# gitvicky/CP-PRE

Hardware: AMD Instinct MI355X
Metric: residual-cells/s (PRE eval+calibrate) (higher is better)
Workload: dtype f32

## Files before the change

### cp_pre_amd/csrc/calib.hip

```cpp
#include "common.h"
#include "guarded_divide.h"

#pragma clang fp contract(off)

namespace {

__global__ void __launch_bounds__(256) absdiff_kernel(const float *__restrict__ a, const float *__restrict__ b,
                                                      float *__restrict__ out, long long n)
{
    const bool vec = !(((uintptr_t)a | (uintptr_t)out | (uintptr_t)(b ? b : a)) & 15);
    long long done = 0;
    if (vec) {
        const long long n4 = n / 4;
        const float4 *a4 = reinterpret_cast<const float4 *>(a);
        const float4 *b4 = reinterpret_cast<const float4 *>(b);
        float4 *o4 = reinterpret_cast<float4 *>(out);
        for (long long blk = blockIdx.x; blk * 1024 < n4; blk += gridDim.x) {
            const long long i = blk * 1024 + threadIdx.x;
            float4 v[4], w[4];
#pragma unroll
            for (int u = 0; u < 4; ++u)
                if (i + u * 256 < n4) v[u] = a4[i + u * 256];
            if (b) {
#pragma unroll
// ... 100 lines not shown
        constexpr int width = 64 * H / US;
#pragma unroll
        for (int k = 0; k < H; ++k) {
            if constexpr (width == 32) {
                const ms_u32x2 r = __builtin_amdgcn_permlane32_swap(m[k], m[H + k], false, false);
                m[k] = max(r.x, r.y);
            } else if constexpr (width == 16) {
                const ms_u32x2 r = __builtin_amdgcn_permlane16_swap(m[k], m[H + k], false, false);
                m[k] = max(r.x, r.y);
            } else {
                const bool up = lane & width;
                const unsigned int mine = up ? m[H + k] : m[k], send = up ? m[k] : m[H + k];
                m[k] = max(mine, dpp_xor<width>(send));
            }
        }
        ms_butterfly<US, H / 2>(m, lane);
    }
}

__device__ __forceinline__ float ms_cell(const float *p, unsigned int cb, unsigned int plane_bytes)
{
    const __amdgpu_buffer_rsrc_t r = __builtin_amdgcn_make_buffer_rsrc(const_cast<float *>(p), 0, plane_bytes, 0x00020000);
    return __uint_as_float(__builtin_amdgcn_raw_buffer_load_b32(r, (int)cb, 0, 0));
}

template <int TCH, int US, bool FULL>
__device__ __forceinline__ void ms_load(const float *__restrict__ au, unsigned int c, long long row_stride, long long plane, int i, int nt,
                                        float (&v)[US][TCH])
{
#pragma unroll
    for (int u = 0; u < US; ++u)
#pragma unroll
        for (int t = 0; t < TCH; ++t)
            v[u][t] = ms_cell(au + ((i + u) * row_stride + (FULL || TCH == 1 || t < nt ? t : nt - 1) * plane), c, (unsigned int)plane * 4u);
}

struct MsStage { unsigned int (*m)[17]; unsigned int *row0; long long nseg_left; };
template <int TCH, int US, bool FULL>
__device__ __forceinline__ void ms_use(const float (&v)[US][TCH], int i, int nt, bool scored, double (&s)[TCH], double (&q)[TCH],
                                       unsigned int *__restrict__ seg, long long seg_stride, const MsStage *stage = nullptr)
{
    unsigned int m[US];
#pragma unroll
    for (int u = 0; u < US; ++u) {
        int mp = 0;
        unsigned int mn = 0u;
#pragma unroll
        for (int t = 0; t < TCH; ++t) {
            const float x = (FULL || TCH == 1 || t < nt) ? v[u][t] : 0.f;
            const double d = (double)x;
            s[t] += d;
            q[t] = __builtin_fma(d, d, q[t]);
            mp = max(mp, (int)__float_as_uint(x));
            mn = max(mn, __float_as_uint(x));
        }
        m[u] = max((unsigned int)mp, mn & 0x7fffffffu);
        m[u] = scored ? m[u] : 0u;
    }
    const int lane = threadIdx.x & 63;
    if constexpr (US == 1) {
        m[0] = wave_max_u32_to_lane63(m[0]);
        if (lane == 63 && seg) seg[i * seg_stride] = m[0];
    } else {
        ms_butterfly<US, US / 2>(m, lane);
        if constexpr (64 / US > 8) m[0] = max(m[0], dpp_xor<8>(m[0]));
        if constexpr (64 / US > 4) m[0] = max(m[0], dpp_xor<4>(m[0]));
        m[0] = max(m[0], dpp_xor<2>(m[0]));
        m[0] = max(m[0], dpp_xor<1>(m[0]));
        if (US == 16 && stage) {
            if ((lane & 3) == 0) stage->m[threadIdx.x >> 6][lane >> 2] = m[0];
            __syncthreads();
            if (threadIdx.x < 256) {
                const int smp = (int)(threadIdx.x >> 4), sg = (int)(threadIdx.x & 15);
                if (sg < stage->nseg_left) stage->row0[(i + smp) * seg_stride + sg] = stage->m[sg][smp];
            }
            __syncthreads();
        } else if ((lane & (64 / US - 1)) == 0) seg[(i + lane / (64 / US)) * seg_stride] = m[0];
    }
}

template <int TCH, int US, bool FULL>
__device__ __forceinline__ void ms_samples(const float *__restrict__ au, unsigned int c, long long row_stride, long long plane, int i0, int i1,
                                           int nt, bool scored, double (&s)[TCH], double (&q)[TCH], unsigned int *__restrict__ seg,
                                           long long seg_stride, const MsStage *stage = nullptr)
{
    int i = i0;
    if constexpr (US == 1) {
        float va[1][TCH], vb[1][TCH];
        if (i < i1) ms_load<TCH, 1, FULL>(au, c, row_stride, plane, i, nt, va);
        for (; i < i1; i += 2) {
            ms_load<TCH, 1, FULL>(au, c, row_stride, plane, min(i + 1, i1 - 1), nt, vb);
            ms_use<TCH, 1, FULL>(va, i, nt, scored, s, q, seg, seg_stride);
            if (i + 1 >= i1) break;
            ms_load<TCH, 1, FULL>(au, c, row_stride, plane, min(i + 2, i1 - 1), nt, va);
            ms_use<TCH, 1, FULL>(vb, i + 1, nt, scored, s, q, seg, seg_stride);
        }
    } else {
        float v[US][TCH], w[US][TCH], v1[1][TCH];
        const int ilast = i0 + (i1 - i0) / US * US - US;
        if (i + US <= i1) ms_load<TCH, US, FULL>(au, c, row_stride, plane, i, nt, v);
        for (; i + US <= i1; i += 2 * US) {
            ms_load<TCH, US, FULL>(au, c, row_stride, plane, min(i + US, ilast), nt, w);
            ms_use<TCH, US, FULL>(v, i, nt, scored, s, q, seg, seg_stride, stage);
            if (i + 2 * US > i1) { i += US; break; }
            ms_load<TCH, US, FULL>(au, c, row_stride, plane, min(i + 2 * US, ilast), nt, v);
            ms_use<TCH, US, FULL>(w, i + US, nt, scored, s, q, seg, seg_stride, stage);
        }
        for (; i < i1; ++i) {
            ms_load<TCH, 1, FULL>(au, c, row_stride, plane, i, nt, v1);
            ms_use<TCH, 1, FULL>(v1, i, nt, scored, s, q, seg, seg_stride);
        }
    }
}

template <int TCH, int US>
__global__ void __launch_bounds__(US == 16 && MS_STAGE ? 1024 : 256)
moments_segmax_kernel(const float *__restrict__ a, long long row_stride, int n, int T, int X,
                                                             int Y, int cx, int cy, int rows_per_split, double *__restrict__ sum,
                                                             double *__restrict__ sumsq, unsigned int *__restrict__ segmax)
{
    const long long plane = (long long)X * Y, cl = (long long)blockIdx.x * blockDim.x + threadIdx.x;
    if (!(US == 16 && MS_STAGE) && (cl & ~63LL) >= plane) return;
    const bool live = cl < plane;
    const long long c = live ? cl : plane - 1;
    const int x = (int)(c / Y), y = (int)(c - (long long)x * Y);
    const long long nseg = (plane + 63) / 64;
    const bool scored = live && x >= cx && x < X - cx && y >= cy && y < Y - cy;
    const int i0 = blockIdx.y * rows_per_split, i1 = min(n, i0 + rows_per_split);
    const int tc = blockIdx.z, TC = gridDim.z, t0 = tc * MS_TMAX, nt = min(TCH, T - t0);
    const float *au = a + (long long)t0 * plane;
    const long long seg_stride = (long long)TC * nseg;
    unsigned int *seg = segmax + (long long)tc * nseg + (cl >> 6);
    double s[TCH], q[TCH];
#pragma unroll
    for (int t = 0; t < TCH; ++t) s[t] = q[t] = 0.0;
    const unsigned int cb = (unsigned int)c * 4u;
    __shared__ unsigned int stage_m[US == 16 ? 16 : 1][17];
    MsStage st{stage_m, segmax + (long long)tc * nseg + (long long)blockIdx.x * (blockDim.x >> 6),
               nseg - (long long)blockIdx.x * (blockDim.x >> 6)};
    const MsStage *stage = (US == 16 && MS_STAGE) ? &st : nullptr;
    if (US == 16 && MS_STAGE && (cl & ~63LL) >= plane) seg = nullptr;
    if (nt == TCH) ms_samples<TCH, US, true>(au, cb, row_stride, plane, i0, i1, nt, scored, s, q, seg, seg_stride, stage);
    else ms_samples<TCH, US, false>(au, cb, row_stride, plane, i0, i1, nt, scored, s, q, seg, seg_stride, stage);
    sum += (long long)t0 * plane + c;
    sumsq += (long long)t0 * plane + c;
#pragma unroll
    for (int t = 0; t < TCH; ++t)
        if (t < nt && live) {
            if (gridDim.y == 1) { sum[t * plane] += s[t]; sumsq[t * plane] += q[t]; }
            else { atomicAdd(&sum[t * plane], s[t]); atomicAdd(&sumsq[t * plane], q[t]); }
        }
}

constexpr int MS4_US = 8;
constexpr int MS4_CG = 4;
constexpr int MS4_NT = 256 * MS4_CG, MS4_NW = 4 * MS4_CG;
constexpr int MS4_WANT = 256;
constexpr int MS4_AUX = 2;
typedef unsigned int ms4_u32x4 __attribute__((ext_vector_type(4)));

__device__ __forceinline__ void ms4_barrier()
{
    __builtin_amdgcn_fence(__ATOMIC_RELEASE, "workgroup", "local");
    __builtin_amdgcn_s_barrier();
    __builtin_amdgcn_fence(__ATOMIC_ACQUIRE, "workgroup", "local");
}

__device__ __forceinline__ void ms4_load(const float *au, unsigned int cb, long long row_stride, long long plane, int i, int nt,
                                         ms4_u32x4 (&v)[4])
{
#pragma unroll
    for (int k = 0; k < 4; ++k) {
        const __amdgpu_buffer_rsrc_t r = __builtin_amdgcn_make_buffer_rsrc(
            const_cast<float *>(au + ((long long)i * row_stride + k * plane)), 0, k < nt ? (unsigned int)plane * 4u : 0u, 0x00020000);
        v[k] = __builtin_amdgcn_raw_buffer_load_b128(r, (int)cb, 0, MS4_AUX);
    }
}

__device__ __forceinline__ unsigned int ms4_use(const ms4_u32x4 (&v)[4], const bool (&scored)[4], double (&s)[4][4], double (&q)[4][4])
{
    unsigned int m = 0u;
#pragma unroll
    for (int j = 0; j < 4; ++j) {
        int mp = 0;
        unsigned int mn = 0u;
#pragma unroll
        for (int k = 0; k < 4; ++k) {
            const unsigned int b = v[k][j];
            const double d = (double)__uint_as_float(b);
            s[k][j] += d;
            q[k][j] = __builtin_fma(d, d, q[k][j]);
            mp = max(mp, (int)b);
            mn = max(mn, b);
        }
        const unsigned int mc = max((unsigned int)mp, mn & 0x7fffffffu);
        m = max(m, scored[j] ? mc : 0u);
    }
    return m;
}

__device__ __forceinline__ void ms4_sample(const ms4_u32x4 (&v)[4], const bool (&scored)[4], double (&s)[4][4], double (&q)[4][4],
                                           unsigned int (&slot)[MS4_NW][4], int w, int lane)
{
    unsigned int m = ms4_use(v, scored, s, q);
    m = max(m, (unsigned int)__builtin_amdgcn_update_dpp(0, (int)m, 0x111, 0xf, 0xf, true));
    m = max(m, (unsigned int)__builtin_amdgcn_update_dpp(0, (int)m, 0x112, 0xf, 0xf, true));
    m = max(m, (unsigned int)__builtin_amdgcn_update_dpp(0, (int)m, 0x114, 0xf, 0xf, true));
    m = max(m, (unsigned int)__builtin_amdgcn_update_dpp(0, (int)m, 0x118, 0xf, 0xf, true));
    if ((lane & 15) == 15) slot[w][lane >> 4] = m;
}

__device__ __forceinline__ void ms4_samples(const float *au, unsigned int cb, long long row_stride, long long plane, int i0, int i1,
                                            int nt, const bool (&scored)[4], double (&s)[4][4], double (&q)[4][4],
                                            unsigned int (*stage)[MS4_US][MS4_NW][4], unsigned int *row0, int nseg_left,
                                            long long seg_stride)
{
    const int w = __builtin_amdgcn_readfirstlane((int)(threadIdx.x >> 6)), lane = (int)(threadIdx.x & 63);
    ms4_u32x4 va[4], vb[4];
    ms4_load(au, cb, row_stride, plane, i0, nt, va);
    int b = 0;
    for (int ib = i0; ib < i1; ib += MS4_US, b ^= 1) {
        const int cnt = min(MS4_US, i1 - ib);
#pragma unroll
        for (int u = 0; u < MS4_US; u += 2) {
            ms4_load(au, cb, row_stride, plane, min(ib + u + 1, i1 - 1), nt, vb);
            if (u < cnt) ms4_sample(va, scored, s, q, stage[b][u], w, lane);
            ms4_load(au, cb, row_stride, plane, min(ib + u + 2, i1 - 1), nt, va);
            if (u + 1 < cnt) ms4_sample(vb, scored, s, q, stage[b][u + 1], w, lane);
        }
        ms4_barrier();
        if (threadIdx.x < MS4_US * MS4_NW) {
            const int smp = (int)(threadIdx.x / MS4_NW), sg = (int)(threadIdx.x % MS4_NW), cg = sg >> 2, r = sg & 3;
            const unsigned int m = max(max(stage[b][smp][4 * cg][r], stage[b][smp][4 * cg + 1][r]),
                                       max(stage[b][smp][4 * cg + 2][r], stage[b][smp][4 * cg + 3][r]));
            if (smp < cnt && sg < nseg_left) row0[(long long)(ib + smp) * seg_stride + sg] = m;
        }
    }
}

__global__ void __launch_bounds__(MS4_NT) moments_segmax4_kernel(const float *__restrict__ a, long long row_stride, int n, int T,
                                                               int X, int Y, int cx, int cy, int rows_per_split,
                                                               double *__restrict__ sum, double *__restrict__ sumsq,
                                                               unsigned int *__restrict__ segmax)
{
    const long long plane = (long long)X * Y;
    const int w = __builtin_amdgcn_readfirstlane((int)(threadIdx.x >> 6)), lane = (int)(threadIdx.x & 63);
    const long long cl = (long long)blockIdx.x * MS4_NT + (w >> 2) * 256 + lane * 4;
    const bool live = cl < plane;
    const long long c = live ? cl : plane - 4;
    bool scored[4];
#pragma unroll
    for (int j = 0; j < 4; ++j) {
        const int x = (int)((c + j) / Y), y = (int)(c + j - (long long)x * Y);
        scored[j] = live && x >= cx && x < X - cx && y >= cy && y < Y - cy;
    }
    const long long nseg = (plane + 63) / 64;
    const int i0 = blockIdx.y * rows_per_split, i1 = min(n, i0 + rows_per_split);
    const int tc = blockIdx.z, TC = gridDim.z, t0 = tc * MS_TMAX + 4 * (w & 3), nt = min(4, T - t0);
    const float *au = a + (long long)min(t0, T - 1) * plane;
    const long long seg_stride = (long long)TC * nseg;
    unsigned int *row0 = segmax + (long long)tc * nseg + (long long)blockIdx.x * MS4_NW;
    const int nseg_left = (int)min((long long)MS4_NW, nseg - (long long)blockIdx.x * MS4_NW);
    double s[4][4], q[4][4];
#pragma unroll
    for (int k = 0; k < 4; ++k)
#pragma unroll
        for (int j = 0; j < 4; ++j) s[k][j] = q[k][j] = 0.0;
    __shared__ unsigned int stage[2][MS4_US][MS4_NW][4];
    const unsigned int cb = (unsigned int)c * 4u;
    ms4_samples(au, cb, row_stride, plane, i0, i1, nt, scored, s, q, stage, row0, nseg_left, seg_stride);
    if (!live) return;
#pragma unroll
    for (int k = 0; k < 4; ++k)
        if (k < nt) {
            double *ps = sum + (long long)(t0 + k) * plane + c, *pq = sumsq + (long long)(t0 + k) * plane + c;
#pragma unroll
            for (int j = 0; j < 4; ++j) {
                if (gridDim.y == 1) { ps[j] += s[k][j]; pq[j] += q[k][j]; }
                else { atomicAdd(&ps[j], s[k][j]); atomicAdd(&pq[j], q[k][j]); }
            }
        }
}

__global__ void __launch_bounds__(256) std_from_moments_kernel(const double *__restrict__ sum, const double *__restrict__ sumsq,
                                                               double n_total, long long M, float eps, float *__restrict__ mod)
{
    const long long c = (long long)blockIdx.x * blockDim.x + threadIdx.x;
    if (c >= M) return;
    const double mean = sum[c] / n_total;
    double var = sumsq[c] / n_total - mean * mean;
    var = var < 0.0 ? 0.0 : var;
    mod[c] = (float)sqrt(var) + eps;
}

__device__ __forceinline__ float wave_max(float v)
{
#pragma unroll
    for (int o = 32; o > 0; o >>= 1) v = fmaxf(v, __shfl_xor(v, o));
    return v;
}

constexpr int JS_RB = 32;
#ifndef JS_TARGET_CELLS
#define JS_TARGET_CELLS 65536
#endif
__device__ __forceinline__ void js_update(float av, float sv, float &m, float &thr, bool &nan)
{
    guarded_max_update(av, sv, m, thr, nan);
}

__global__ void __launch_bounds__(256) joint_score_kernel(const float *__restrict__ a, const float *__restrict__ b,
                                                          const float *__restrict__ mod, int T, int X, int Y,
                                                          int ct, int cx, int cy, int groups, int smp_fastest,
                                                          const unsigned int *__restrict__ only, float *__restrict__ scores)
{
    const long long plane = (long long)X * Y, vol = plane * T;
    const int smp = smp_fastest ? blockIdx.x : blockIdx.y;
    const unsigned int cblk = smp_fastest ? blockIdx.y : blockIdx.x;
    if (only && !only[smp]) return;
    const float *pa = a + smp * vol, *pb = b ? b + smp * vol : nullptr;
    const long long nrows = (long long)T * X;
    const bool vec = (Y % 4 == 0) && !(((uintptr_t)a | (uintptr_t)mod | (uintptr_t)(b ? b : a)) & 15);
    __shared__ unsigned int rowmask;
    __shared__ float red[4];
    float m = 0.f, thr = 0.f;
    bool any = false, nan = false;
    for (int gi = 0; gi < groups; ++gi) {
    const long long r0 = ((long long)cblk * groups + gi) * JS_RB;
    if (r0 >= nrows) break;
    __syncthreads();
    if (threadIdx.x < 64) {
        const long long r = r0 + threadIdx.x;
        bool ok = threadIdx.x < JS_RB && r < nrows;
        if (ok) {
            const int t = (int)(r / X), x = (int)(r % X);
            ok = !(t < ct || t >= T - ct || x < cx || x >= X - cx);
        }
        const unsigned long long bm = __ballot(ok);
        if (threadIdx.x == 0) rowmask = (unsigned int)bm;
    }
    __syncthreads();
    const unsigned int rows = rowmask;
    any = any || rows != 0u;
    if (rows && vec) {
        const int Y4 = Y / 4, dr = 256 / Y4, dy = 256 % Y4;
        int row = threadIdx.x / Y4, y4 = threadIdx.x % Y4;
        while (row < JS_RB) {
            if ((rows >> row) & 1u) {
                const long long o = (r0 + row) * Y + 4 * y4;
                float4 v = *reinterpret_cast<const float4 *>(pa + o);
                if (pb) { const float4 w = *reinterpret_cast<const float4 *>(pb + o); v = make_float4(v.x - w.x, v.y - w.y, v.z - w.z, v.w - w.w); }
                const float4 sg = *reinterpret_cast<const float4 *>(mod + o);
                const float av[4] = {fabsf(v.x), fabsf(v.y), fabsf(v.z), fabsf(v.w)};
                const float sv[4] = {sg.x, sg.y, sg.z, sg.w};
                const int y = 4 * y4;
#pragma unroll
                for (int k = 0; k < 4; ++k)
                    if (y + k >= cy && y + k < Y - cy) js_update(av[k], sv[k], m, thr, nan);
            }
            y4 += dy;
            row += dr;
            if (y4 >= Y4) { y4 -= Y4; ++row; }
        }
    } else if (rows) {
        const int dr = 256 / Y, dy = 256 % Y;
        int row = threadIdx.x / Y, y = threadIdx.x % Y;
        while (row < JS_RB) {
            if (((rows >> row) & 1u) && y >= cy && y < Y - cy) {
                const long long o = (r0 + row) * Y + y;
                float v = pa[o];
                if (pb) v -= pb[o];
                js_update(fabsf(v), mod[o], m, thr, nan);
            }
            y += dy;
            row += dr;
            if (y >= Y) { y -= Y; ++row; }
        }
    }
    }
    m = wave_max(m);
    if (__ballot(nan)) m = __uint_as_float(0x7fc00000u);
    if ((threadIdx.x & 63) == 0) red[threadIdx.x >> 6] = m;
    __syncthreads();
    if (threadIdx.x == 0 && any) {
        const unsigned int u = max(max(__float_as_uint(red[0]), __float_as_uint(red[1])),
                                   max(__float_as_uint(red[2]), __float_as_uint(red[3])));
        atomicMax(reinterpret_cast<unsigned int *>(scores) + smp, u);
    }
}

constexpr int JSF_CELLS = 8192;
__global__ void __launch_bounds__(256) joint_score_flat_kernel(const float *__restrict__ a, const float *__restrict__ b,
                                                               const float *__restrict__ mod, int T, int X, int Y, int ct,
                                                               int cx, int cy, const unsigned int *__restrict__ only,
                                                               float *__restrict__ scores)
{
    const long long vol = (long long)T * X * Y;
    const int smp = blockIdx.x;
    if (only && !only[smp]) return;
    const float4 *pa = reinterpret_cast<const float4 *>(a + smp * vol);
    const float4 *pb = b ? reinterpret_cast<const float4 *>(b + smp * vol) : nullptr;
    const float4 *pm = reinterpret_cast<const float4 *>(mod);
    const unsigned int c0 = blockIdx.y * (unsigned)JSF_CELLS;
    __shared__ float red[4];
    float m = 0.f, thr = 0.f;
    bool nan = false;
    unsigned int f = c0 + 4u * threadIdx.x;
    const unsigned int row0 = f / (unsigned)Y;
    int y0 = (int)(f - row0 * (unsigned)Y), x0 = (int)(row0 % (unsigned)X), t0 = (int)(row0 / (unsigned)X);
    const int dy = 1024 % Y, drow = 1024 / Y, dx = drow % X, dt = drow / X;
    for (int k = 0; k < JSF_CELLS / 1024 && f < (unsigned)vol; ++k, f += 1024u) {
        float4 v = pa[f >> 2];
        if (pb) { const float4 w = pb[f >> 2]; v = make_float4(v.x - w.x, v.y - w.y, v.z - w.z, v.w - w.w); }
        const float4 sg = pm[f >> 2];
        const float av[4] = {fabsf(v.x), fabsf(v.y), fabsf(v.z), fabsf(v.w)};
        const float sv[4] = {sg.x, sg.y, sg.z, sg.w};
        int y = y0, x = x0, t = t0;
#pragma unroll
        for (int j = 0; j < 4; ++j) {
            const bool in = t >= ct && t < T - ct && x >= cx && x < X - cx && y >= cy && y < Y - cy;
            if (in) js_update(av[j], sv[j], m, thr, nan);
            if (++y == Y) { y = 0; if (++x == X) { x = 0; ++t; } }
        }
        y0 += dy;
        const int carry = y0 >= Y;
        y0 -= carry ? Y : 0;
        x0 += dx + carry;
        const int cx2 = x0 >= X;
        x0 -= cx2 ? X : 0;
        t0 += dt + cx2;
    }
    m = wave_max(m);
    if (__ballot(nan)) m = __uint_as_float(0x7fc00000u);
    if ((threadIdx.x & 63) == 0) red[threadIdx.x >> 6] = m;
// ... 198 lines not shown
                } else if (hit) {
                    atomicAdd(&hist[d], 1u);
                }
            }
        };
        const float4 *s4 = reinterpret_cast<const float4 *>(s);
        for (long long i = threadIdx.x; i < N8; i += blockDim.x) {
            const float4 a = s4[2 * i], b = s4[2 * i + 1];
            count(a.x); count(a.y); count(a.z); count(a.w);
            count(b.x); count(b.y); count(b.z); count(b.w);
        }
        for (long long i = 8 * N8 + threadIdx.x; i < N; i += blockDim.x) count(s[i]);
        __syncthreads();
        if (threadIdx.x < 64) {
            const unsigned int c0 = hist[4 * lane], c1 = hist[4 * lane + 1], c2 = hist[4 * lane + 2], c3 = hist[4 * lane + 3];
            long long incl = (long long)c0 + c1 + c2 + c3;
#pragma unroll
            for (int o = 1; o < 64; o <<= 1) {
                const long long up = __shfl_up(incl, o);
                if (lane >= o) incl += up;
            }
            long long excl = incl - ((long long)c0 + c1 + c2 + c3);
            const bool mine = (excl <= rank && rank < incl) || (lane == 63 && rank >= incl);
            if (mine) {
                unsigned int d = 4 * lane;
                if (rank >= excl + c0) { excl += c0; ++d; if (rank >= excl + c1) { excl += c1; ++d; if (rank >= excl + c2) { excl += c2; ++d; } } }
                sh_prefix = prefix | (d << shift);
                sh_rank = rank - excl;
            }
        }
        __syncthreads();
        prefix = sh_prefix;
        rank = sh_rank;
        mask |= 255u << shift;
        __syncthreads();
    }
    if (threadIdx.x == 0) out[j] = sh_nan ? __uint_as_float(0x7fc00000u) : key2f(prefix);
}

__global__ void __launch_bounds__(256) cov_count_kernel(const float *__restrict__ y, const float *__restrict__ lo,
                                                        const float *__restrict__ hi, long long total, long long M,
                                                        int per_sample, unsigned long long *count)
{
    unsigned int local = 0;
    for (long long i = (long long)blockIdx.x * blockDim.x + threadIdx.x; i < total; i += (long long)gridDim.x * blockDim.x) {
        const long long c = per_sample ? i : i % M;
        const float v = y[i];
        local += (v >= lo[c]) && (v <= hi[c]);
    }
#pragma unroll
    for (int o = 32; o > 0; o >>= 1) local += __shfl_xor(local, o);
    __shared__ unsigned int red[4];
    if ((threadIdx.x & 63) == 0) red[threadIdx.x >> 6] = local;
    __syncthreads();
    if (threadIdx.x == 0) atomicAdd(count, (unsigned long long)(red[0] + red[1] + red[2] + red[3]));
}

__global__ void __launch_bounds__(256) cov_count4_kernel(const float4 *__restrict__ y, const float4 *__restrict__ lo,
                                                         const float4 *__restrict__ hi, int n, long long M4, int per_sample,
                                                         int rows_per, unsigned long long *count)
{
    const long long q = (long long)blockIdx.x * blockDim.x + threadIdx.x;
    unsigned int local = 0;
    if (q < M4) {
        const int s0 = blockIdx.y * rows_per, s1 = min(n, s0 + rows_per);
        float4 l = lo[q], h = hi[q];
        auto inside = [&](const float4 &v, const float4 &a, const float4 &b) __attribute__((always_inline)) {
            return (unsigned)((v.x >= a.x) && (v.x <= b.x)) + (unsigned)((v.y >= a.y) && (v.y <= b.y)) +
                   (unsigned)((v.z >= a.z) && (v.z <= b.z)) + (unsigned)((v.w >= a.w) && (v.w <= b.w));
        };
        int s = s0;
        if (!per_sample) {
            for (; s + 7 < s1; s += 8) {
                float4 v[8];
#pragma unroll
                for (int u = 0; u < 8; ++u) v[u] = y[(long long)(s + u) * M4 + q];
#pragma unroll
                for (int u = 0; u < 8; ++u) local += inside(v[u], l, h);
            }
        }
        for (; s < s1; ++s) {
            const long long o = (long long)s * M4 + q;
            if (per_sample) { l = lo[o]; h = hi[o]; }
            local += inside(y[o], l, h);
        }
    }
#pragma unroll
    for (int o = 32; o > 0; o >>= 1) local += __shfl_xor(local, o);
    __shared__ unsigned int red[4];
    if ((threadIdx.x & 63) == 0) red[threadIdx.x >> 6] = local;
    __syncthreads();
    if (threadIdx.x == 0 && (red[0] | red[1] | red[2] | red[3])) atomicAdd(count, (unsigned long long)(red[0] + red[1] + red[2] + red[3]));
}

__global__ void __launch_bounds__(256) cov_joint_kernel(const float *__restrict__ y, const float *__restrict__ lo,
                                                        const float *__restrict__ hi, long long M, int per_sample,
                                                        uint8_t *inside)
{
    const int smp = blockIdx.y;
    const float *py = y + smp * M;
    const float *plo = lo + (per_sample ? smp * M : 0), *phi = hi + (per_sample ? smp * M : 0);
    bool bad = false;
    if (M % 4 == 0 && !(((uintptr_t)y | (uintptr_t)lo | (uintptr_t)hi) & 15)) {
        const float4 *y4 = reinterpret_cast<const float4 *>(py), *l4 = reinterpret_cast<const float4 *>(plo),
                     *h4 = reinterpret_cast<const float4 *>(phi);
        for (long long q = (long long)blockIdx.x * blockDim.x + threadIdx.x; q < M / 4; q += (long long)gridDim.x * blockDim.x) {
            const float4 v = y4[q], a = l4[q], b = h4[q];
            bad |= !((v.x >= a.x) && (v.x <= b.x) && (v.y >= a.y) && (v.y <= b.y) && (v.z >= a.z) && (v.z <= b.z) &&
                     (v.w >= a.w) && (v.w <= b.w));
        }
    } else {
        for (long long c = (long long)blockIdx.x * blockDim.x + threadIdx.x; c < M; c += (long long)gridDim.x * blockDim.x) {
            const float v = py[c];
            bad |= !((v >= plo[c]) && (v <= phi[c]));
        }
    }
    if (__any(bad) && (threadIdx.x & 63) == 0) inside[smp] = 0;
}

__global__ void __launch_bounds__(256) cov_rowcount_kernel(const float *__restrict__ y, const float *__restrict__ lo,
                                                           const float *__restrict__ hi, long long M, int per_sample,
                                                           int outside, unsigned int *__restrict__ counts)
{
    const int smp = blockIdx.y;
    const float *py = y + smp * M;
    const float *plo = lo + (per_sample ? smp * M : 0), *phi = hi + (per_sample ? smp * M : 0);
    unsigned int local = 0;
    auto hit = [&](float v, float a, float b) __attribute__((always_inline)) {
        return (unsigned)(outside ? ((v <= a) || (v >= b)) : ((v >= a) && (v <= b)));
    };
    if (M % 4 == 0 && !(((uintptr_t)y | (uintptr_t)lo | (uintptr_t)hi) & 15)) {
        const float4 *y4 = reinterpret_cast<const float4 *>(py), *l4 = reinterpret_cast<const float4 *>(plo),
                     *h4 = reinterpret_cast<const float4 *>(phi);
        for (long long q = (long long)blockIdx.x * blockDim.x + threadIdx.x; q < M / 4; q += (long long)gridDim.x * blockDim.x) {
            const float4 v = y4[q], a = l4[q], b = h4[q];
            local += hit(v.x, a.x, b.x) + hit(v.y, a.y, b.y) + hit(v.z, a.z, b.z) + hit(v.w, a.w, b.w);
        }
    } else {
        for (long long c = (long long)blockIdx.x * blockDim.x + threadIdx.x; c < M; c += (long long)gridDim.x * blockDim.x)
            local += hit(py[c], plo[c], phi[c]);
    }
#pragma unroll
    for (int o = 32; o > 0; o >>= 1) local += __shfl_xor(local, o);
    if ((threadIdx.x & 63) == 0 && local) atomicAdd(counts + smp, local);
}

inline unsigned grid_for(long long items, int block, long long cap = 256LL * 32)
{
    long long g = (items + block - 1) / block;
    if (g < 1) g = 1;
    return (unsigned)(g > cap ? cap : g);
}

}

extern "C" {

int pre_absdiff_f32(const float *a, const float *b, float *out, int64_t n, void *stream)
{
    if (!a || !out || n < 0) return PRE_E_NULL;
    if (n == 0) return PRE_OK;
    hipLaunchKernelGGL(absdiff_kernel, dim3(grid_for(n / 16 + 1, 256, 0x7fffffffLL)), dim3(256), 0, as_stream(stream), a, b, out, (long long)n);
    PRE_LAUNCH_CHECK();
    return PRE_OK;
}

int pre_std_axis0_f32(const float *a, const float *b, int64_t n, int64_t M, float eps, float *mod, void *stream)
{
    if (!a || !mod || n <= 0 || M <= 0) return PRE_E_NULL;
    if (n > 0x7fffffff || M > 0xffffff00LL) return PRE_E_SHAPE;
    const int bs = M >= (1 << 19) ? 256 : 64;
    hipLaunchKernelGGL(std_axis0_kernel, dim3((unsigned)((M + bs - 1) / bs)), dim3(bs), 0, as_stream(stream), a, b, (int)n,
                       (long long)M, eps, mod);
    PRE_LAUNCH_CHECK();
    return PRE_OK;
}

int pre_moments_axis0_f64(const float *a, const float *b, int64_t n, int64_t M, int64_t row_stride, double *sum,
                          double *sumsq, void *stream)
{
    if (!a || !sum || !sumsq || n <= 0 || M <= 0 || row_stride < M) return PRE_E_NULL;
    if (n > 0x7fffffff || M > 0xffffff00LL) return PRE_E_SHAPE;
    const long long bx = (M + 255) / 256;
    long long splits = 1;
    while (bx * splits < 1024 && splits * 32 < n) splits *= 2;
    const int rows = (int)((n + splits - 1) / splits);
    splits = (n + rows - 1) / rows;
    hipLaunchKernelGGL(moments_kernel, dim3((unsigned)bx, (unsigned)splits), dim3(256), 0, as_stream(stream), a, b, (int)n,
                       (long long)M, (long long)row_stride, rows, sum, sumsq);
    PRE_LAUNCH_CHECK();
    return PRE_OK;
}

int pre_moments_segmax_f64(const float *a, int64_t row_stride, int64_t n, int64_t T, int64_t X, int64_t Y, int crop_x, int crop_y,
                           double *sum, double *sumsq, uint32_t *segmax, void *stream)
{
    if (!a || !sum || !sumsq || !segmax || n <= 0 || T <= 0 || X <= 0 || Y <= 0) return PRE_E_NULL;
    if (crop_x < 0 || crop_y < 0 || row_stride < T * X * Y) return PRE_E_RANGE;
    const int us = T == 1 ? 16 : T <= 4 ? 4 : 1;
    if (us == 1 && (X * Y) % 4 == 0 && row_stride % 4 == 0 && !((uintptr_t)a & 15)) {
        const long long bx = (X * Y + MS4_NT - 1) / MS4_NT, TC = (T + MS_TMAX - 1) / MS_TMAX;
        if (n > 0x7fffffff || bx > 0x7fffffffLL || TC > 65535 || T > 0x7fffffff) return PRE_E_SHAPE;
        if (X * Y >= (1LL << 30)) return PRE_E_SHAPE;
        long long splits = 1;
        while (bx * TC * splits < MS4_WANT && splits * 32 < n) splits *= 2;
        const int rows = (int)((n + splits - 1) / splits);
        splits = (n + rows - 1) / rows;
        hipLaunchKernelGGL(moments_segmax4_kernel, dim3((unsigned)bx, (unsigned)splits, (unsigned)TC), dim3(MS4_NT), 0,
                           as_stream(stream), a, (long long)row_stride, (int)n, (int)T, (int)X, (int)Y, crop_x, crop_y, rows, sum,
                           sumsq, segmax);
        PRE_LAUNCH_CHECK();
        return PRE_OK;
    }
    const int bt = (us == 16 && MS_STAGE) ? 1024 : 256;
    const long long bx = (X * Y + bt - 1) / bt, TC = (T + MS_TMAX - 1) / MS_TMAX;
    if (n > 0x7fffffff || bx > 0x7fffffffLL || TC > 65535 || T > 0x7fffffff) return PRE_E_SHAPE;
    if (X * Y >= (1LL << 30)) return PRE_E_SHAPE;
    long long splits = 1;
    const long long want = us == 16 ? 16384 : us > 1 ? 2048 : MS_WANT1;
    while (bx * (bt / 256) * TC * splits < want && splits * 32 * us < n) splits *= 2;
    const int rows = (int)((n + splits - 1) / splits);
    splits = (n + rows - 1) / rows;
    const dim3 grid((unsigned)bx, (unsigned)splits, (unsigned)TC);
#define PRE_MS_LAUNCH(TCH, US)                                                                                                \
    hipLaunchKernelGGL((moments_segmax_kernel<TCH, US>), grid, dim3(bt), 0, as_stream(stream), a, (long long)row_stride, (int)n,    \
                       (int)T, (int)X, (int)Y, crop_x, crop_y, rows, sum, sumsq, segmax)
    if (us == 16) PRE_MS_LAUNCH(1, 16);
    else if (us == 4) PRE_MS_LAUNCH(4, 4);
    else PRE_MS_LAUNCH(MS_TMAX, 1);
#undef PRE_MS_LAUNCH
    PRE_LAUNCH_CHECK();
    return PRE_OK;
}

int pre_std_from_moments_f32(const double *sum, const double *sumsq, int64_t n_total, int64_t M, float eps, float *mod,
                             void *stream)
{
    if (!sum || !sumsq || !mod || n_total <= 0 || M <= 0) return PRE_E_NULL;
    if (M > 0xffffff00LL) return PRE_E_SHAPE;
    hipLaunchKernelGGL(std_from_moments_kernel, dim3((unsigned)((M + 255) / 256)), dim3(256), 0, as_stream(stream), sum, sumsq,
                       (double)n_total, (long long)M, eps, mod);
    PRE_LAUNCH_CHECK();
    return PRE_OK;
}

static int joint_score_launch(const float *a, const float *b, const float *mod, int64_t n, int64_t T, int64_t X, int64_t Y,
                              int crop_t, int crop_x, int crop_y, const uint32_t *only, float *scores, void *stream)
{
    if (!a || !mod || !scores || n <= 0 || T <= 0 || X <= 0 || Y <= 0) return PRE_E_NULL;
    if (crop_t < 0 || crop_x < 0 || crop_y < 0) return PRE_E_RANGE;
    if (n > 65535 * 1024LL || T * X > 0x7fffffffLL * JS_RB || Y > 0x7fffffff) return PRE_E_SHAPE;
    {
        const long long vol = (long long)T * X * Y, nblk = (vol + JSF_CELLS - 1) / JSF_CELLS;
        if (Y < 64 && vol % 4 == 0 && vol < 0x7fffffffLL && nblk <= 65535 && n <= 0x7fffffff &&
            !(((uintptr_t)a | (uintptr_t)mod | (uintptr_t)(b ? b : a)) & 15)) {
            hipLaunchKernelGGL(joint_score_flat_kernel, dim3((unsigned)n, (unsigned)nblk), dim3(256), 0, as_stream(stream), a, b, mod,
                               (int)T, (int)X, (int)Y, crop_t, crop_x, crop_y, only, scores);
            PRE_LAUNCH_CHECK();
            return PRE_OK;
        }
    }
    const long long spans = (T * X + JS_RB - 1) / JS_RB;
    long long groups = JS_TARGET_CELLS / (JS_RB * Y);
    if (groups < 1) groups = 1;
    while (groups > 1 && (spans / groups) * n < 2048) groups /= 2;
    const long long chunks = (spans + groups - 1) / groups;
    for (int64_t s0 = 0; s0 < n; s0 += 65535) {
        const int64_t ns = (n - s0) < 65535 ? (n - s0) : 65535;
        const long long vol = (long long)T * X * Y;
        const int swap = chunks <= 65535;
        hipLaunchKernelGGL(joint_score_kernel, swap ? dim3((unsigned)ns, (unsigned)chunks) : dim3((unsigned)chunks, (unsigned)ns),
                           dim3(256), 0, as_stream(stream), a + s0 * vol, b ? b + s0 * vol : nullptr, mod, (int)T, (int)X, (int)Y,
                           crop_t, crop_x, crop_y, (int)groups, swap, only ? only + s0 : nullptr, scores + s0);
        PRE_LAUNCH_CHECK();
    }
    return PRE_OK;
}

int pre_joint_score_f32(const float *a, const float *b, const float *mod, int64_t n, int64_t T, int64_t X, int64_t Y,
                        int crop_t, int crop_x, int crop_y, float *scores, void *stream)
{
    return joint_score_launch(a, b, mod, n, T, X, Y, crop_t, crop_x, crop_y, nullptr, scores, stream);
}

int pre_joint_score_flagged_f32(const float *a, const float *b, const float *mod, int64_t n, int64_t T, int64_t X, int64_t Y,
                                int crop_t, int crop_x, int crop_y, const uint32_t *flags, float *scores, void *stream)
{
    if (!flags) return PRE_E_NULL;
    return joint_score_launch(a, b, mod, n, T, X, Y, crop_t, crop_x, crop_y, flags, scores, stream);
}

int pre_segmin_mod_f32(const float *mod, int64_t T, int64_t X, int64_t Y, int crop_x, int crop_y, float *segmin, void *stream)
{
    if (!mod || !segmin || T <= 0 || X <= 0 || Y <= 0) return PRE_E_NULL;
    if (crop_x < 0 || crop_y < 0) return PRE_E_RANGE;
    const long long nseg = (X * Y + JP_SEG - 1) / JP_SEG, TC = (T + MS_TMAX - 1) / MS_TMAX;
    if (X > 0x7fffffff || Y > 0x7fffffff || nseg > 0x7fffffffLL || TC > 65535) return PRE_E_SHAPE;
    hipLaunchKernelGGL(segmin_kernel, dim3((unsigned)nseg, (unsigned)TC), dim3(64), 0, as_stream(stream), mod, (int)T, (int)X, (int)Y,
                       crop_x, crop_y, nseg, segmin);
    PRE_LAUNCH_CHECK();
    return PRE_OK;
}

static int pruned_lds_max()
{
    int dev = 0, lds_max = 0;
    if (hipGetDevice(&dev) != hipSuccess ||
        hipDeviceGetAttribute(&lds_max, hipDeviceAttributeMaxSharedMemoryPerBlock, dev) != hipSuccess || lds_max <= 0) {
        (void)hipGetLastError();
        lds_max = 64 * 1024;
    }
    return lds_max;
}

int64_t pre_joint_score_pruned_max_segments(void) { return (pruned_lds_max() - 256) / 4; }

int pre_joint_score_pruned_f32(const float *res, int64_t row_stride, const float *mod, const uint32_t *segmax, const float *segmin,
                               int64_t n, int64_t T, int64_t X, int64_t Y, int crop_x, int crop_y, float *scores,
                               uint32_t *flags, unsigned long long *stats, void *stream)
{
    if (!res || !mod || !segmax || !segmin || !scores || n <= 0 || T <= 0 || X <= 0 || Y <= 0) return PRE_E_NULL;
    if (crop_x < 0 || crop_y < 0 || row_stride < T * X * Y) return PRE_E_RANGE;
    const long long nseg = (X * Y + JP_SEG - 1) / JP_SEG, TC = (T + MS_TMAX - 1) / MS_TMAX, total = TC * nseg;
    if (n > 0x7fffffff || T > 0x7fffffff || X > 0x7fffffff || Y > 0x7fffffff) return PRE_E_SHAPE;
    const int lds_max = pruned_lds_max();
    if (total * 4 + 256 > lds_max) return PRE_E_UNSUPPORTED;
    if (total * 4 + 256 > 64 * 1024) {
        if (hipFuncSetAttribute(reinterpret_cast<const void *>(joint_score_pruned_kernel<false>), hipFuncAttributeMaxDynamicSharedMemorySize,
                                lds_max - 256) != hipSuccess) {
            (void)hipGetLastError();
            return PRE_E_UNSUPPORTED;
        }
    }
    if (n >= 4096 && total <= 2048) {
        hipLaunchKernelGGL(joint_score_pruned_kernel<true>, dim3((unsigned)((n + 3) / 4)), dim3(256), (size_t)total * 16,
                           as_stream(stream), res, (long long)row_stride, mod, segmax, segmin, (int)n, (int)T, (int)X, (int)Y, crop_x,
                           crop_y, (int)nseg, (int)total, scores, flags, stats);
        PRE_LAUNCH_CHECK();
        return PRE_OK;
    }
    const int threads = n >= 2048 ? 256 : n >= 512 ? 512 : 1024;
    hipLaunchKernelGGL(joint_score_pruned_kernel<false>, dim3((unsigned)n), dim3(threads), (size_t)total * 4, as_stream(stream), res,
                       (long long)row_stride, mod, segmax, segmin, (int)n, (int)T, (int)X, (int)Y, crop_x, crop_y, (int)nseg, (int)total,
                       scores, flags, stats);
    PRE_LAUNCH_CHECK();
    return PRE_OK;
}

int pre_kth_f32(const float *scores, int64_t N, const int64_t *ks, int nk, float *out, void *stream)
{
    if (!scores || !ks || !out || N <= 0 || nk <= 0) return PRE_E_NULL;
    for (int j = 0; j < nk; ++j)
        if (ks[j] < 0 || ks[j] >= N) return PRE_E_RANGE;
    for (int j0 = 0; j0 < nk; j0 += 16) {
        KList kl;
        kl.nk = (nk - j0) < 16 ? (nk - j0) : 16;
        for (int j = 0; j < kl.nk; ++j) kl.k[j] = ks[j0 + j];
        hipLaunchKernelGGL(kth_kernel, dim3(kl.nk), dim3(1024), 0, as_stream(stream), scores, (long long)N, kl, out + j0);
        PRE_LAUNCH_CHECK();
    }
    return PRE_OK;
}

int pre_cov_count_f32(const float *y, const float *lo, const float *hi, int64_t n, int64_t M, int per_sample_bounds,
                      unsigned long long *count, void *stream)
{
// ... 53 lines not shown
```

Before: 300.7 billion.

## Generalize moments_segmax4 kernel over time-width and route small-T and axis0 moments through it

Templates the vectorized buffer-load moments/segmax kernel on per-wave time width, waves per group, and samples per load batch, with a compile-time switch to drop the segmax reduction. Small-T cases (T<=4) now use the float4 buffer-load path with multiple samples in flight per load instead of the older scalar kernels. Plain axis-0 moments also reuse this kernel without segmax when aligned. The aim is higher memory-level parallelism and less instruction overhead per cell. In exchange, templates and register pressure grow, and the split heuristic changes for the PW=1 variants.

```diff
diff --git a/cp_pre_amd/csrc/calib.hip b/cp_pre_amd/csrc/calib.hip
--- a/cp_pre_amd/csrc/calib.hip
+++ b/cp_pre_amd/csrc/calib.hip
@@ -276,12 +276,17 @@
         }
 }
 
-constexpr int MS4_US = 8;
 constexpr int MS4_CG = 4;
-constexpr int MS4_NT = 256 * MS4_CG, MS4_NW = 4 * MS4_CG;
+constexpr int MS4_CELLS = 256 * MS4_CG;
 constexpr int MS4_WANT = 256;
+constexpr int MS4_SW_FEW = 4;
 constexpr int MS4_AUX = 2;
 typedef unsigned int ms4_u32x4 __attribute__((ext_vector_type(4)));
+template <int PG, int SW> struct Ms4Geom {
+    static constexpr int NW = PG * MS4_CG, NT = 64 * NW;
+    static constexpr int US = SW > 4 ? 2 * SW : 8;
+    static_assert(US % (2 * SW) == 0 && US * 4 * MS4_CG <= NT, "one thread per sample and segment after the barrier");
+};
 
 __device__ __forceinline__ void ms4_barrier()
 {
@@ -290,18 +295,22 @@
     __builtin_amdgcn_fence(__ATOMIC_ACQUIRE, "workgroup", "local");
 }
 
-__device__ __forceinline__ void ms4_load(const float *au, unsigned int cb, long long row_stride, long long plane, int i, int nt,
-                                         ms4_u32x4 (&v)[4])
-{
-#pragma unroll
-    for (int k = 0; k < 4; ++k) {
-        const __amdgpu_buffer_rsrc_t r = __builtin_amdgcn_make_buffer_rsrc(
-            const_cast<float *>(au + ((long long)i * row_stride + k * plane)), 0, k < nt ? (unsigned int)plane * 4u : 0u, 0x00020000);
-        v[k] = __builtin_amdgcn_raw_buffer_load_b128(r, (int)cb, 0, MS4_AUX);
-    }
-}
-
-__device__ __forceinline__ unsigned int ms4_use(const ms4_u32x4 (&v)[4], const bool (&scored)[4], double (&s)[4][4], double (&q)[4][4])
+template <int PW, int SW>
+__device__ __forceinline__ void ms4_load(const float *au, unsigned int cb, long long row_stride, long long plane, int i, int ilast,
+                                         const unsigned int (&nb)[PW], ms4_u32x4 (&v)[PW * SW])
+{
+#pragma unroll
+    for (int u = 0; u < SW; ++u)
+#pragma unroll
+        for (int k = 0; k < PW; ++k) {
+            const __amdgpu_buffer_rsrc_t r = __builtin_amdgcn_make_buffer_rsrc(
+                const_cast<float *>(au + ((long long)min(i + u, ilast) * row_stride + k * plane)), 0, nb[k], 0x00020000);
+            v[u * PW + k] = __builtin_amdgcn_raw_buffer_load_b128(r, (int)cb, 0, MS4_AUX);
+        }
+}
+
+template <int PW, bool SEGMAX>
+__device__ __forceinline__ unsigned int ms4_use(const ms4_u32x4 *v, const bool (&scored)[4], double (&s)[PW][4], double (&q)[PW][4])
 {
     unsigned int m = 0u;
 #pragma unroll
@@ -309,101 +318,133 @@
         int mp = 0;
         unsigned int mn = 0u;
 #pragma unroll
-        for (int k = 0; k < 4; ++k) {
+        for (int k = 0; k < PW; ++k) {
             const unsigned int b = v[k][j];
             const double d = (double)__uint_as_float(b);
             s[k][j] += d;
             q[k][j] = __builtin_fma(d, d, q[k][j]);
-            mp = max(mp, (int)b);
-            mn = max(mn, b);
-        }
-        const unsigned int mc = max((unsigned int)mp, mn & 0x7fffffffu);
-        m = max(m, scored[j] ? mc : 0u);
+            if constexpr (SEGMAX) {
+                mp = max(mp, (int)b);
+                mn = max(mn, b);
+            }
+        }
+        if constexpr (SEGMAX) {
+            const unsigned int mc = max((unsigned int)mp, mn & 0x7fffffffu);
+            m = max(m, scored[j] ? mc : 0u);
+        }
     }
     return m;
 }
 
-__device__ __forceinline__ void ms4_sample(const ms4_u32x4 (&v)[4], const bool (&scored)[4], double (&s)[4][4], double (&q)[4][4],
-                                           unsigned int (&slot)[MS4_NW][4], int w, int lane)
-{
-    unsigned int m = ms4_use(v, scored, s, q);
-    m = max(m, (unsigned int)__builtin_amdgcn_update_dpp(0, (int)m, 0x111, 0xf, 0xf, true));
-    m = max(m, (unsigned int)__builtin_amdgcn_update_dpp(0, (int)m, 0x112, 0xf, 0xf, true));
-    m = max(m, (unsigned int)__builtin_amdgcn_update_dpp(0, (int)m, 0x114, 0xf, 0xf, true));
-    m = max(m, (unsigned int)__builtin_amdgcn_update_dpp(0, (int)m, 0x118, 0xf, 0xf, true));
-    if ((lane & 15) == 15) slot[w][lane >> 4] = m;
-}
-
+template <int PW, bool SEGMAX>
+__device__ __forceinline__ void ms4_sample(const ms4_u32x4 *v, const bool (&scored)[4], double (&s)[PW][4], double (&q)[PW][4],
+                                           unsigned int (*slot)[4], int w, int lane)
+{
+    unsigned int m = ms4_use<PW, SEGMAX>(v, scored, s, q);
+    if constexpr (SEGMAX) {
+        m = max(m, (unsigned int)__builtin_amdgcn_update_dpp(0, (int)m, 0x111, 0xf, 0xf, true));
+        m = max(m, (unsigned int)__builtin_amdgcn_update_dpp(0, (int)m, 0x112, 0xf, 0xf, true));
+        m = max(m, (unsigned int)__builtin_amdgcn_update_dpp(0, (int)m, 0x114, 0xf, 0xf, true));
+        m = max(m, (unsigned int)__builtin_amdgcn_update_dpp(0, (int)m, 0x118, 0xf, 0xf, true));
+        if ((lane & 15) == 15) slot[w][lane >> 4] = m;
+    }
+}
+
+template <int PW, int PG, int SW, bool SEGMAX>
 __device__ __forceinline__ void ms4_samples(const float *au, unsigned int cb, long long row_stride, long long plane, int i0, int i1,
-                                            int nt, const bool (&scored)[4], double (&s)[4][4], double (&q)[4][4],
-                                            unsigned int (*stage)[MS4_US][MS4_NW][4], unsigned int *row0, int nseg_left,
-                                            long long seg_stride)
-{
+                                            const unsigned int (&nb)[PW], const bool (&scored)[4], double (&s)[PW][4],
+                                            double (&q)[PW][4], unsigned int (*stage)[Ms4Geom<PG, SW>::US][Ms4Geom<PG, SW>::NW][4],
+                                            unsigned int *row0, int nseg_left, long long seg_stride)
+{
+    constexpr int US = Ms4Geom<PG, SW>::US;
     const int w = __builtin_amdgcn_readfirstlane((int)(threadIdx.x >> 6)), lane = (int)(threadIdx.x & 63);
-    ms4_u32x4 va[4], vb[4];
-    ms4_load(au, cb, row_stride, plane, i0, nt, va);
+    ms4_u32x4 va[PW * SW], vb[PW * SW];
+    ms4_load<PW, SW>(au, cb, row_stride, plane, i0, i1 - 1, nb, va);
     int b = 0;
-    for (int ib = i0; ib < i1; ib += MS4_US, b ^= 1) {
-        const int cnt = min(MS4_US, i1 - ib);
-#pragma unroll
-        for (int u = 0; u < MS4_US; u += 2) {
-            ms4_load(au, cb, row_stride, plane, min(ib + u + 1, i1 - 1), nt, vb);
-            if (u < cnt) ms4_sample(va, scored, s, q, stage[b][u], w, lane);
-            ms4_load(au, cb, row_stride, plane, min(ib + u + 2, i1 - 1), nt, va);
-            if (u + 1 < cnt) ms4_sample(vb, scored, s, q, stage[b][u + 1], w, lane);
-        }
-        ms4_barrier();
-        if (threadIdx.x < MS4_US * MS4_NW) {
-            const int smp = (int)(threadIdx.x / MS4_NW), sg = (int)(threadIdx.x % MS4_NW), cg = sg >> 2, r = sg & 3;
-            const unsigned int m = max(max(stage[b][smp][4 * cg][r], stage[b][smp][4 * cg + 1][r]),
-                                       max(stage[b][smp][4 * cg + 2][r], stage[b][smp][4 * cg + 3][r]));
-            if (smp < cnt && sg < nseg_left) row0[(long long)(ib + smp) * seg_stride + sg] = m;
-        }
-    }
-}
-
-__global__ void __launch_bounds__(MS4_NT) moments_segmax4_kernel(const float *__restrict__ a, long long row_stride, int n, int T,
-                                                               int X, int Y, int cx, int cy, int rows_per_split,
-                                                               double *__restrict__ sum, double *__restrict__ sumsq,
-                                                               unsigned int *__restrict__ segmax)
-{
+    for (int ib = i0; ib < i1; ib += US, b ^= 1) {
+        const int cnt = min(US, i1 - ib);
+#pragma unroll
+        for (int u = 0; u < US; u += 2 * SW) {
+            ms4_load<PW, SW>(au, cb, row_stride, plane, ib + u + SW, i1 - 1, nb, vb);
+#pragma unroll
+            for (int x = 0; x < SW; ++x)
+                if (u + x < cnt) ms4_sample<PW, SEGMAX>(va + x * PW, scored, s, q, SEGMAX ? stage[b][u + x] : nullptr, w, lane);
+            ms4_load<PW, SW>(au, cb, row_stride, plane, ib + u + 2 * SW, i1 - 1, nb, va);
+#pragma unroll
+            for (int x = 0; x < SW; ++x)
+                if (u + SW + x < cnt) ms4_sample<PW, SEGMAX>(vb + x * PW, scored, s, q, SEGMAX ? stage[b][u + SW + x] : nullptr, w, lane);
+        }
+        if constexpr (SEGMAX) {
+            ms4_barrier();
+            if (threadIdx.x < US * 4 * MS4_CG) {
+                const int smp = (int)(threadIdx.x / (4 * MS4_CG)), sg = (int)(threadIdx.x % (4 * MS4_CG)), cg = sg >> 2, r = sg & 3;
+                unsigned int m = stage[b][smp][PG * cg][r];
+#pragma unroll
+                for (int g = 1; g < PG; ++g) m = max(m, stage[b][smp][PG * cg + g][r]);
+                if (smp < cnt && sg < nseg_left) row0[(long long)(ib + smp) * seg_stride + sg] = m;
+            }
+        }
+    }
+}
+
+template <int PW, int PG, int SW, bool SEGMAX>
+__global__ void __launch_bounds__((Ms4Geom<PG, SW>::NT)) moments_segmax4_kernel(const float *__restrict__ a, long long row_stride, int n,
+                                                                            int T, int X, int Y, long long cells, int cx, int cy,
+                                                                            int rows_per_split, double *__restrict__ sum,
+                                                                            double *__restrict__ sumsq,
+                                                                            unsigned int *__restrict__ segmax)
+{
+    using G = Ms4Geom<PG, SW>;
     const long long plane = (long long)X * Y;
     const int w = __builtin_amdgcn_readfirstlane((int)(threadIdx.x >> 6)), lane = (int)(threadIdx.x & 63);
-    const long long cl = (long long)blockIdx.x * MS4_NT + (w >> 2) * 256 + lane * 4;
+    const long long cl = (long long)blockIdx.x * MS4_CELLS + (w / PG) * 256 + lane * 4;
     const bool live = cl < plane;
     const long long c = live ? cl : plane - 4;
     bool scored[4];
 #pragma unroll
     for (int j = 0; j < 4; ++j) {
-        const int x = (int)((c + j) / Y), y = (int)(c + j - (long long)x * Y);
-        scored[j] = live && x >= cx && x < X - cx && y >= cy && y < Y - cy;
+        if constexpr (SEGMAX) {
+            const int x = (int)((c + j) / Y), y = (int)(c + j - (long long)x * Y);
+            scored[j] = live && x >= cx && x < X - cx && y >= cy && y < Y - cy;
+        } else scored[j] = false;
     }
     const long long nseg = (plane + 63) / 64;
     const int i0 = blockIdx.y * rows_per_split, i1 = min(n, i0 + rows_per_split);
-    const int tc = blockIdx.z, TC = gridDim.z, t0 = tc * MS_TMAX + 4 * (w & 3), nt = min(4, T - t0);
+    const int tc = blockIdx.z, TC = gridDim.z, t0 = tc * MS_TMAX + PW * (w % PG);
     const float *au = a + (long long)min(t0, T - 1) * plane;
+    unsigned int nb[PW];
+#pragma unroll
+    for (int k = 0; k < PW; ++k)
+        nb[k] = t0 + k < T ? (unsigned int)min(plane, cells - (long long)(t0 + k) * plane) * 4u : 0u;
     const long long seg_stride = (long long)TC * nseg;
-    unsigned int *row0 = segmax + (long long)tc * nseg + (long long)blockIdx.x * MS4_NW;
-    const int nseg_left = (int)min((long long)MS4_NW, nseg - (long long)blockIdx.x * MS4_NW);
-    double s[4][4], q[4][4];
-#pragma unroll
-    for (int k = 0; k < 4; ++k)
+    unsigned int *row0 = SEGMAX ? segmax + (long long)tc * nseg + (long long)blockIdx.x * (4 * MS4_CG) : nullptr;
+    const int nseg_left = (int)min((long long)(4 * MS4_CG), nseg - (long long)blockIdx.x * (4 * MS4_CG));
+    double s[PW][4], q[PW][4];
+#pragma unroll
+    for (int k = 0; k < PW; ++k)
 #pragma unroll
         for (int j = 0; j < 4; ++j) s[k][j] = q[k][j] = 0.0;
-    __shared__ unsigned int stage[2][MS4_US][MS4_NW][4];
+    unsigned int (*stage)[G::US][G::NW][4] = nullptr;
+    if constexpr (SEGMAX) {
+        __shared__ unsigned int stage_m[2][G::US][G::NW][4];
+        stage = stage_m;
+    }
     const unsigned int cb = (unsigned int)c * 4u;
-    ms4_samples(au, cb, row_stride, plane, i0, i1, nt, scored, s, q, stage, row0, nseg_left, seg_stride);
+    ms4_samples<PW, PG, SW, SEGMAX>(au, cb, row_stride, plane, i0, i1, nb, scored, s, q,
+                                    stage, row0, nseg_left, seg_stride);
     if (!live) return;
 #pragma unroll
-    for (int k = 0; k < 4; ++k)
-        if (k < nt) {
-            double *ps = sum + (long long)(t0 + k) * plane + c, *pq = sumsq + (long long)(t0 + k) * plane + c;
+    for (int k = 0; k < PW; ++k) {
+        const long long c0 = (long long)(t0 + k) * plane + c;
+        if (t0 + k < T && c0 < cells) {
+            double *ps = sum + c0, *pq = sumsq + c0;
 #pragma unroll
             for (int j = 0; j < 4; ++j) {
                 if (gridDim.y == 1) { ps[j] += s[k][j]; pq[j] += q[k][j]; }
                 else { atomicAdd(&ps[j], s[k][j]); atomicAdd(&pq[j], q[k][j]); }
             }
         }
+    }
 }
 
 __global__ void __launch_bounds__(256) std_from_moments_kernel(const double *__restrict__ sum, const double *__restrict__ sumsq,
@@ -908,6 +949,28 @@
     return (unsigned)(g > cap ? cap : g);
 }
 
+template <int PW, int PG, int SW, bool SEGMAX>
+int ms4_launch(const float *a, long long row_stride, long long n, long long T, long long X, long long Y, long long cells, int cx,
+               int cy, double *sum, double *sumsq, uint32_t *segmax, void *stream)
+{
+    const long long bx = (X * Y + MS4_CELLS - 1) / MS4_CELLS, TC = (T + MS_TMAX - 1) / MS_TMAX;
+    if (n > 0x7fffffff || bx > 0x7fffffffLL || TC > 65535 || T > 0x7fffffff) return PRE_E_SHAPE;
+    if (X * Y >= (1LL << 30)) return PRE_E_SHAPE;
+    long long splits = 1;
+    if (PW == 1) {
+        splits = MS4_WANT * 16 / Ms4Geom<PG, SW>::NW / (bx * TC);
+        if (splits > (n + 31) / 32) splits = (n + 31) / 32;
+        if (splits < 1) splits = 1;
+    } else while (bx * TC * splits < MS4_WANT && splits * 32 < n) splits *= 2;
+    const int rows = (int)((n + splits - 1) / splits);
+    splits = (n + rows - 1) / rows;
+    hipLaunchKernelGGL((moments_segmax4_kernel<PW, PG, SW, SEGMAX>), dim3((unsigned)bx, (unsigned)splits, (unsigned)TC),
+                       dim3(Ms4Geom<PG, SW>::NT), 0, as_stream(stream), a, row_stride, (int)n, (int)T, (int)X, (int)Y, cells, cx, cy,
+                       rows, sum, sumsq, segmax);
+    PRE_LAUNCH_CHECK();
+    return PRE_OK;
+}
+
 }
 
 extern "C" {
@@ -937,6 +1000,9 @@
 {
     if (!a || !sum || !sumsq || n <= 0 || M <= 0 || row_stride < M) return PRE_E_NULL;
     if (n > 0x7fffffff || M > 0xffffff00LL) return PRE_E_SHAPE;
+    if (!b && M % 4 == 0 && row_stride % 4 == 0 && !((uintptr_t)a & 15) && M <= 65535LL * MS_TMAX * MS4_CELLS)
+        return ms4_launch<4, 4, 1, false>(a, row_stride, n, (M + MS4_CELLS - 1) / MS4_CELLS, 1, MS4_CELLS, M, 0, 0, sum, sumsq,
+                                          nullptr, stream);
     const long long bx = (M + 255) / 256;
     long long splits = 1;
     while (bx * splits < 1024 && splits * 32 < n) splits *= 2;
@@ -953,21 +1019,16 @@
 {
     if (!a || !sum || !sumsq || !segmax || n <= 0 || T <= 0 || X <= 0 || Y <= 0) return PRE_E_NULL;
     if (crop_x < 0 || crop_y < 0 || row_stride < T * X * Y) return PRE_E_RANGE;
+    if ((X * Y) % 4 == 0 && row_stride % 4 == 0 && !((uintptr_t)a & 15)) {
+#define PRE_MS4_LAUNCH(PW, PG, SW)                                                                                              \
+    return ms4_launch<PW, PG, SW, true>(a, row_stride, n, T, X, Y, T * X * Y, crop_x, crop_y, sum, sumsq, segmax, stream)
+        if (T > 4) PRE_MS4_LAUNCH(4, 4, 1);
+        if (T > 2) PRE_MS4_LAUNCH(1, 4, MS4_SW_FEW);
+        if (T > 1) PRE_MS4_LAUNCH(1, 2, MS4_SW_FEW);
+        PRE_MS4_LAUNCH(1, 1, MS4_SW_FEW);
+#undef PRE_MS4_LAUNCH
+    }
     const int us = T == 1 ? 16 : T <= 4 ? 4 : 1;
-    if (us == 1 && (X * Y) % 4 == 0 && row_stride % 4 == 0 && !((uintptr_t)a & 15)) {
-        const long long bx = (X * Y + MS4_NT - 1) / MS4_NT, TC = (T + MS_TMAX - 1) / MS_TMAX;
-        if (n > 0x7fffffff || bx > 0x7fffffffLL || TC > 65535 || T > 0x7fffffff) return PRE_E_SHAPE;
-        if (X * Y >= (1LL << 30)) return PRE_E_SHAPE;
-        long long splits = 1;
-        while (bx * TC * splits < MS4_WANT && splits * 32 < n) splits *= 2;
-        const int rows = (int)((n + splits - 1) / splits);
-        splits = (n + rows - 1) / rows;
-        hipLaunchKernelGGL(moments_segmax4_kernel, dim3((unsigned)bx, (unsigned)splits, (unsigned)TC), dim3(MS4_NT), 0,
-                           as_stream(stream), a, (long long)row_stride, (int)n, (int)T, (int)X, (int)Y, crop_x, crop_y, rows, sum,
-                           sumsq, segmax);
-        PRE_LAUNCH_CHECK();
-        return PRE_OK;
-    }
     const int bt = (us == 16 && MS_STAGE) ? 1024 : 256;
     const long long bx = (X * Y + bt - 1) / bt, TC = (T + MS_TMAX - 1) / MS_TMAX;
     if (n > 0x7fffffff || bx > 0x7fffffffLL || TC > 65535 || T > 0x7fffffff) return PRE_E_SHAPE;
```

Measured after the change: 300.4 billion. No clear change (-0.1%).
